# iacopoermacora/Street-sparse-3DGS

Hardware: AMD Instinct MI355X
Metric: fwd+bwd Mpix/s at 1080p (1M Gaussians) (higher is better)
Workload: dtype f32; 1 GPU; rasterizer fwd+bwd, 1000000 Gaussians, SH degree 3, 1920x1080, do_depth; gaussians=1000000, width=1920, height=1080, sh_degree=3, tiles=8160, fwd_segment=2048, parallelism=chunk-per-gpu x1

## Files before the change

street-sparse-3dgs_amd/csrc/dsort.hip:

```cpp
#include "gsr_launch.h"

namespace gsr {

namespace {

constexpr int kDsThreads = 1024;
constexpr int kDsWaves = kDsThreads / kWave;
constexpr int kDsItems = 8;
constexpr int kDsTile = kDsThreads * kDsItems;
constexpr int kDigitBits = 9;
constexpr int kRadix = 1 << kDigitBits;
constexpr int kPasses = 4;
constexpr int kLookWin = 16;
constexpr int kMaxResident = 240;
constexpr uint32_t kKeyBase = 0x3E4CCCCDu;
constexpr uint32_t kTopNarrow = 32u;

constexpr int kCtlTicket = 0;
constexpr int kCtlDone = 4;
constexpr int kCtlK = 5;
constexpr int kCtlErr = 6;
constexpr int kCtlAux = 7;
constexpr int kCtlMaxSB = 8;
constexpr int kCtlFwdReady = 9;
constexpr int kCtlSpare = 10;
constexpr int kCtlCulled = 12;
constexpr int kCtlLive = 13;
constexpr int kCtlWide = 15;
constexpr int kCtlHead = 16;
constexpr int kUpMax = 128;
constexpr int kRowVec = 4;
constexpr int kRowSets = kDsThreads / (kRadix / kRowVec);
constexpr int kRowLoads = kUpMax / kRowSets;
constexpr int kRowGroup = 8;
__host__ __device__ inline int up_tpb(int nb) { return (nb + kUpMax - 1) / kUpMax; }
__host__ __device__ inline int up_blocks(int nb) { return (nb + up_tpb(nb) - 1) / up_tpb(nb); }
__host__ __device__ inline size_t ctl_status(int nb, int p) { return kCtlHead + (size_t)p * nb * kRadix; }
__host__ __device__ inline size_t ctl_zero_words(int nb) { return ctl_status(nb, kPasses); }
__host__ __device__ inline size_t ctl_bex(int nb) { return ctl_zero_words(nb); }
__host__ __device__ inline size_t ctl_btot(int nb) { return ctl_bex(nb) + nb; }
__host__ __device__ inline size_t ctl_blkhist(int nb) { return (ctl_btot(nb) + kUpMax + 63) / 64 * 64; }
__host__ __device__ inline size_t ctl_words(int nb) { return ctl_blkhist(nb) + (size_t)kUpMax * kPasses * kRadix; }
constexpr int kSpinLimit = 1 << 20;

#ifdef GSR_DS_TRACE
__device__ uint64_t *g_ds_trace;
#define DS_STAMP(kern, slot)                                                                          \
    do {                                                                                              \
        if (threadIdx.x == 0) {                                                                       \
            const uint64_t t_ = __builtin_amdgcn_s_memrealtime();                                     \
            __builtin_amdgcn_s_waitcnt(0xC07F);                                                       \
            if (blockIdx.x < 4096) g_ds_trace[((size_t)(kern) * 4096 + blockIdx.x) * 8 + (slot)] = t_; \
        }                                                                                             \
    } while (0)
#else
#define DS_STAMP(kern, slot) \
    do {                     \
    } while (0)
#endif
#ifdef GSR_DS_TRACE
#define DS_STAMP_AFTER(kern, slot, x)            \
    do {                                         \
        asm volatile("s_waitcnt vmcnt(0)" ::"v"(x)); \
        DS_STAMP(kern, slot);                    \
    } while (0)
#else
#define DS_STAMP_AFTER(kern, slot, x) DS_STAMP(kern, slot)
#endif


constexpr uint32_t kFlagAgg = 1u << 30, kFlagInc = 2u << 30, kCountMask = (1u << 30) - 1u;

__device__ __forceinline__ uint32_t ld_agent(const uint32_t *p) {
    return __hip_atomic_load(p, __ATOMIC_RELAXED, __HIP_MEMORY_SCOPE_AGENT);
}
__device__ __forceinline__ void st_agent(uint32_t *p, uint32_t v) {
    __hip_atomic_store(p, v, __ATOMIC_RELAXED, __HIP_MEMORY_SCOPE_AGENT);
}

__device__ __forceinline__ uint32_t below(uint64_t m) {
    return __builtin_amdgcn_mbcnt_hi((uint32_t)(m >> 32), __builtin_amdgcn_mbcnt_lo((uint32_t)m, 0u));
}

template <int p>
__device__ __forceinline__ uint32_t digit_of(uint32_t key) {
    const uint32_t r = key - kKeyBase;
    if (p < kPasses - 1) return (r >> (kDigitBits * p)) & (uint32_t)(kRadix - 1);
    return (r >> (kDigitBits * p)) + (key >= kKeyBase ? kTopNarrow : 0u);
}

__device__ __forceinline__ uint64_t match_digit(uint32_t d, uint64_t valid) {
    uint64_t m = valid;
#pragma unroll
    for (int b = 0; b < kDigitBits; b++) {
        const uint32_t spread = (uint32_t)((int32_t)(d << (31 - b)) >> 31);
        const uint64_t bb = __ballot(spread != 0u);
        m &= ~(bb ^ ((uint64_t)spread << 32 | spread));
    }
    return m;
}

__device__ __forceinline__ uint32_t wave_incl_scan(uint32_t v, int lane) {
#pragma unroll
    for (int o = 1; o < 64; o <<= 1) {
        const uint32_t t = (uint32_t)__shfl_up((int)v, o, 64);
        if (lane >= o) v += t;
    }
    return v;
}

__device__ __forceinline__ uint32_t scan_radix_wave(uint32_t *a, int lane) {
    constexpr int kPer = kRadix / kWave;
    uint32_t x[kPer], s = 0;
#pragma unroll
    for (int k = 0; k < kPer; k++) {
        x[k] = a[kPer * lane + k];
        s += x[k];
    }
    const uint32_t incl = wave_incl_scan(s, lane);
    uint32_t e = incl - s;
#pragma unroll
    for (int k = 0; k < kPer; k++) {
        a[kPer * lane + k] = e;
        e += x[k];
    }
    return (uint32_t)__shfl((int)incl, 63, 64);
}

__global__ __launch_bounds__(kDsThreads) void dsort_upsweep_kernel(int P, int nb, const uint32_t *__restrict__ keys,
                                                                    const uint32_t *__restrict__ tiles,
                                                                    uint32_t *__restrict__ ctl,
                                                                    uint32_t *__restrict__ host_K,
                                                                    uint32_t *__restrict__ host_wide) {
    GSR_KS(kKsUpsweep);
    constexpr int kMidCopies = 16;
    __shared__ uint32_t s_hist[kPasses * kRadix];
    __shared__ uint32_t s_mid[kMidCopies][kRadix];
    __shared__ uint32_t s_wsum[kDsWaves];
    __shared__ uint32_t s_cull, s_far;
    const int t = threadIdx.x, w = t >> 6, lane = t & 63;
    const int u = blockIdx.x, tpb = up_tpb(nb);
    DS_STAMP(0, 0);
#pragma unroll
    for (int k = 0; k < kPasses * kRadix / kDsThreads; k++) s_hist[t + k * kDsThreads] = 0u;
    if (t == 0) s_cull = s_far = 0u;
#pragma unroll
    for (int k = 0; k < kMidCopies * kRadix / kDsThreads; k++) (&s_mid[0][0])[t + k * kDsThreads] = 0u;
    __syncthreads();
    uint32_t run = 0;
    uint32_t culled = 0;
    uint32_t near = 0;
    bool far = false;
    const int v1 = min(nb, (u + 1) * tpb);
    for (int v = u * tpb; v < v1; v++) {
        const size_t base = (size_t)v * kDsTile + (size_t)w * kDsItems * kWave;
        uint32_t key[kDsItems], tl[kDsItems];
#pragma unroll
        for (int k = 0; k < kDsItems; k++) {
            const size_t e = base + (size_t)k * kWave + lane;
            key[k] = e < (size_t)P ? keys[e] : 0u;
            tl[k] = e < (size_t)P ? tiles[e] : 0u;
        }
        uint32_t sum = 0;
#pragma unroll
        for (int k = 0; k < kDsItems; k++) {
            const size_t e = base + (size_t)k * kWave + lane;
            const bool cull = e < (size_t)P && key[k] == 0xFFFFFFFFu;
            const bool vis = e < (size_t)P && !cull;
            const uint32_t top = digit_of<3>(key[k]);
            const uint64_t nearm = __ballot(vis && top == kTopNarrow);
            culled += (uint32_t)__popcll(__ballot(cull));
            near += (uint32_t)__popcll(nearm);
            if (vis) {
                atomicAdd(&s_hist[digit_of<0>(key[k])], 1u);
                atomicAdd(&s_hist[kRadix + digit_of<1>(key[k])], 1u);
                atomicAdd(&s_mid[lane & (kMidCopies - 1)][digit_of<2>(key[k])], 1u);
                if (top != kTopNarrow) atomicAdd(&s_hist[3 * kRadix + top], 1u);
            }
            far = far || __ballot(vis) != nearm;
            sum += tl[k];
        }
#pragma unroll
        for (int o = 32; o > 0; o >>= 1) sum += (uint32_t)__shfl_xor((int)sum, o, 64);
        if (lane == 0) s_wsum[w] = sum;
        __syncthreads();
        if (t == 0) {
            ctl[ctl_bex(nb) + v] = run;
#pragma unroll
            for (int k = 0; k < kDsWaves; k++) run += s_wsum[k];
        }
        __syncthreads();
    }
    if (lane == 0) {
        if (culled) atomicAdd(&s_cull, culled);
        if (near) atomicAdd(&s_hist[3 * kRadix + kTopNarrow], near);
        if (far) s_far = 1u;
    }
    __syncthreads();
    DS_STAMP(0, 1);
#pragma unroll
    for (int k = 0; k < kPasses * kRadix / kDsThreads; k++) {
        const int i = t + k * kDsThreads;
        uint32_t hv = s_hist[i];
        if (i >= 2 * kRadix && i < 3 * kRadix) {
#pragma unroll
            for (int c = 0; c < kMidCopies; c++) hv += s_mid[c][i - 2 * kRadix];
        }
        ctl[ctl_blkhist(nb) + (size_t)u * kPasses * kRadix + i] = hv;
    }
    if (t == 0) {
        ctl[ctl_btot(nb) + u] = run;
        __hip_atomic_fetch_add(&ctl[kCtlK], run, __ATOMIC_RELAXED, __HIP_MEMORY_SCOPE_AGENT);
        if (s_cull) __hip_atomic_fetch_add(&ctl[kCtlCulled], s_cull, __ATOMIC_RELAXED, __HIP_MEMORY_SCOPE_AGENT);
        if (s_far) __hip_atomic_fetch_or(&ctl[kCtlWide], 1u, __ATOMIC_RELAXED, __HIP_MEMORY_SCOPE_AGENT);
        const uint32_t done = __hip_atomic_fetch_add(&ctl[kCtlDone], 1u, __ATOMIC_ACQ_REL, __HIP_MEMORY_SCOPE_AGENT);
        if (done == (uint32_t)gridDim.x - 1u && host_K) {
            const uint32_t K = ld_agent(&ctl[kCtlK]);
            if (host_wide) __hip_atomic_store(host_wide, ld_agent(&ctl[kCtlWide]), __ATOMIC_RELAXED, __HIP_MEMORY_SCOPE_SYSTEM);
            __hip_atomic_store(host_K, K, __ATOMIC_RELEASE, __HIP_MEMORY_SCOPE_SYSTEM);
        }
    }
    DS_STAMP(0, 2);
}

template <int kPass>
__global__ __launch_bounds__(kDsThreads) void dsort_pass_kernel(int P, int nb, const uint32_t *__restrict__ kin,
                                                                 uint32_t *__restrict__ kout,
                                                                 const uint32_t *__restrict__ vin,
                                                                 uint32_t *__restrict__ vout,
                                                                 uint32_t *__restrict__ order, uint32_t *__restrict__ ctl,
                                                                 uint32_t *__restrict__ offsets,
                                                                 const uint32_t *__restrict__ tiles,
                                                                 const uint2 *__restrict__ rect8,
                                                                 const uint32_t *__restrict__ rect4,
                                                                 uint2 *__restrict__ drect,
                                                                 const uint32_t *__restrict__ rin,
                                                                 uint32_t *__restrict__ rout,
                                                                 uint32_t *__restrict__ host_err) {
    GSR_KS(kKsPass0 + kPass);
    constexpr bool kFirst = kPass == 0;
    const bool wide = kPass >= 2 && ctl[kCtlWide] != 0u;
    if (kPass == kPasses - 1 && !wide) return;
    const bool last = kPass == kPasses - 1 || (kPass == kPasses - 2 && !wide);
    const bool carry = rect4 != nullptr;
    __shared__ uint32_t s_key[kDsTile];
    __shared__ uint32_t s_val[kDsTile];
    __shared__ uint32_t s_rc[kDsTile];
    __shared__ uint32_t s_wh[kDsWaves][kRadix];
    __shared__ __attribute__((aligned(16))) uint32_t s_gb[kRowSets][kRadix];
    __shared__ uint32_t s_bex[kRadix];
    __shared__ uint32_t s_dst[kRadix];
    __shared__ uint32_t s_wsum[kDsWaves];
    __shared__ uint32_t s_v, s_pre, s_nsort;
    const int t = threadIdx.x, w = t >> 6, lane = t & 63;
    DS_STAMP(1 + kPass, 0);
#pragma unroll
    for (int k = 0; k < kDsWaves * kRadix / kDsThreads; k++) (&s_wh[0][0])[t + k * kDsThreads] = 0u;
    const int nbu = up_blocks(nb);
    const uint4 *bh = reinterpret_cast<const uint4 *>(ctl + ctl_blkhist(nb) + kPass * kRadix) + (t & (kRadix / kRowVec - 1));
    const auto row = [&](int q) {
        const int j = t / (kRadix / kRowVec) + kRowSets * q;
        return j < nbu ? bh[(size_t)j * (kPasses * kRadix / kRowVec)] : make_uint4(0u, 0u, 0u, 0u);
    };
    constexpr int kRowGroups = kRowLoads / kRowGroup, kRowEvery = kDsItems / kRowGroups;
    static_assert(kRowLoads % kRowGroup == 0 && kDsItems % kRowGroups == 0, "row groups spread over the ranked items");
    uint4 h[kRowGroup], gsum = make_uint4(0u, 0u, 0u, 0u);
    const auto sum_rows = [&]() {
#pragma unroll
        for (int q = 0; q < kRowGroup; q++) {
            gsum.x += h[q].x;
            gsum.y += h[q].y;
            gsum.z += h[q].z;
            gsum.w += h[q].w;
        }
    };
#pragma unroll
    for (int q = 0; q < kRowGroup; q++) h[q] = row(q);
    uint32_t v = blockIdx.x;
    if (nb > kMaxResident) {
        if (t == 0) s_v = atomicAdd(&ctl[kCtlTicket + kPass], 1u);
        __syncthreads();
        v = s_v;
    } else {
        __builtin_amdgcn_s_waitcnt(0xc07f);
        __builtin_amdgcn_s_barrier();
    }
    const size_t Pn = kFirst ? (size_t)P : (size_t)P - min((size_t)ctl[kCtlCulled], (size_t)P);
    const uint32_t nbv = (uint32_t)((Pn + kDsTile - 1) / kDsTile);
    if (v >= nbv) return;
    DS_STAMP(1 + kPass, 5);
    const int wbase = w * kDsItems * kWave;
    const size_t tile0 = (size_t)v * kDsTile;
    const int n = (int)min((size_t)kDsTile, Pn - tile0);
    uint32_t key[kDsItems], val[kDsItems], tl[kDsItems];
#pragma unroll
    for (int k = 0; k < kDsItems; k++) {
        const int i = wbase + k * kWave + lane;
        const bool valid = i < n;
        key[k] = valid ? kin[tile0 + i] : 0xFFFFFFFFu;
        val[k] = (!kFirst && valid) ? vin[tile0 + i] : 0u;
        tl[k] = (kFirst && valid) ? tiles[tile0 + i] : 0u;
    }
    DS_STAMP_AFTER(1 + kPass, 6, key[kDsItems - 1] + val[kDsItems - 1]);
    if (kFirst) {
        if (w == 0) {
            const int u = (int)v / up_tpb(nb);
            uint32_t c = 0;
#pragma unroll
            for (int q = 0; q < kUpMax / kWave; q++) c += lane + q * kWave < u ? ctl[ctl_btot(nb) + lane + q * kWave] : 0u;
#pragma unroll
            for (int o = 32; o > 0; o >>= 1) c += (uint32_t)__shfl_xor((int)c, o, 64);
            if (lane == 0) s_pre = c + ctl[ctl_bex(nb) + v];
        }
        uint32_t run = 0;
#pragma unroll
        for (int k = 0; k < kDsItems; k++) {
            const uint32_t incl = wave_incl_scan(tl[k], lane);
            s_key[wbase + k * kWave + lane] = run + incl - tl[k];
            run += (uint32_t)__shfl((int)incl, 63, 64);
        }
        if (lane == 0) s_wsum[w] = run;
    }
    uint32_t rk[kDsItems];
#pragma unroll
    for (int k = 0; k < kDsItems; k++) {
        const bool valid = wbase + k * kWave + lane < n && key[k] != 0xFFFFFFFFu;
        const uint32_t d = digit_of<kPass>(key[k]) & (uint32_t)(kRadix - 1);
        const uint64_t m = match_digit(d, __ballot(valid));
        const uint32_t b = below(m);
        const uint32_t old = s_wh[w][d];
        if (valid && b == 0u) s_wh[w][d] = old + (uint32_t)__popcll(m);
        rk[k] = old + b;
        if ((k + 1) % kRowEvery == 0 && (k + 1) / kRowEvery < kRowGroups) {
            asm volatile("" ::: "memory");
            sum_rows();
#pragma unroll
            for (int q = 0; q < kRowGroup; q++) h[q] = row((k + 1) / kRowEvery * kRowGroup + q);
        }
    }
    sum_rows();
    *reinterpret_cast<uint4 *>(&s_gb[t / (kRadix / kRowVec)][kRowVec * (t & (kRadix / kRowVec - 1))]) = gsum;
    uint32_t rc[kDsItems];
    if (carry) {
        const uint32_t *rsrc = kFirst ? rect4 : rin;
#pragma unroll
        for (int k = 0; k < kDsItems; k++) {
            const int i = wbase + k * kWave + lane;
            rc[k] = i < n ? rsrc[tile0 + i] : 0u;
        }
    }
    __syncthreads();
    DS_STAMP(1 + kPass, 1);
    if (kFirst) {
        uint32_t pre = s_pre;
        for (int k = 0; k < w; k++) pre += s_wsum[k];
#pragma unroll
        for (int k = 0; k < kDsItems; k++) {
            const int i = wbase + k * kWave + lane;
            if (i < n) offsets[tile0 + i] = pre + s_key[i];
        }
    }
    uint32_t cnt = 0;
    if (t < kRadix) {
#pragma unroll
        for (int ww = 0; ww < kDsWaves; ww++) {
            const uint32_t c = s_wh[ww][t];
            s_wh[ww][t] = cnt;
            cnt += c;
        }
        uint32_t *st = ctl + ctl_status(nb, kPass);
        st_agent(&st[(size_t)v * kRadix + t], (v == 0 ? kFlagInc : kFlagAgg) | cnt);
        s_bex[t] = cnt;
        uint32_t gb = s_gb[0][t];
#pragma unroll
        for (int q = 1; q < kRowSets; q++) gb += s_gb[q][t];
        s_gb[0][t] = gb;
    }
    __syncthreads();
    if (w == 0) {
        const uint32_t nv = scan_radix_wave(s_bex, lane);
        if (lane == 0) s_nsort = nv;
    }
    if (w == 1) (void)scan_radix_wave(s_gb[0], lane);
    __syncthreads();
    const int nsort = (int)s_nsort;
    DS_STAMP(1 + kPass, 2);
    int wb = wbase + lane;
    asm volatile("" : "+v"(wb));
#pragma unroll
    for (int k = 0; k < kDsItems; k++) {
        const int i = wb + k * kWave;
        if (i < n && key[k] != 0xFFFFFFFFu) {
            const uint32_t d = digit_of<kPass>(key[k]) & (uint32_t)(kRadix - 1);
            const uint32_t lp = s_bex[d] + s_wh[w][d] + rk[k];
            s_key[lp] = key[k];
            s_val[lp] = kFirst ? (uint32_t)tile0 + (uint32_t)i : val[k];
            if (carry) s_rc[lp] = rc[k];
        }
    }
    DS_STAMP(1 + kPass, 7);
    if (t < kRadix) {
        const uint32_t *st = ctl + ctl_status(nb, kPass);
        uint32_t excl = 0;
        int spins = 0;
        for (int j = (int)v - 1; j >= 0;) {
            uint32_t s[kLookWin];
#pragma unroll
            for (int q = 0; q < kLookWin; q++)
                s[q] = j - q >= 0 ? ld_agent(&st[(size_t)(j - q) * kRadix + t]) : kFlagInc;
            int q = 0;
            bool inc = false;
#pragma unroll
            for (int qq = 0; qq < kLookWin; qq++) {
                const uint32_t f = s[qq] & ~kCountMask;
                if (q == qq && f != 0u && !inc) {
                    excl += s[qq] & kCountMask;
                    inc = f == kFlagInc;
                    q = qq + 1;
                }
            }
            if (inc) break;
            j -= q;
            if (q < kLookWin) {
                if (++spins > kSpinLimit) {
                    ctl[kCtlErr] = 1u;
                    if (host_err) __hip_atomic_store(host_err, 1u, __ATOMIC_RELAXED, __HIP_MEMORY_SCOPE_SYSTEM);
                    break;
                }
                __builtin_amdgcn_s_sleep(1);
            }
        }
        if (v > 0) st_agent(&ctl[ctl_status(nb, kPass) + (size_t)v * kRadix + t], kFlagInc | (excl + cnt));
        s_dst[t] = s_gb[0][t] + excl - s_bex[t];
    }
    __syncthreads();
    DS_STAMP(1 + kPass, 3);
    for (int i = t; i < nsort; i += kDsThreads) {
        const uint32_t k = s_key[i];
        const uint32_t j = s_dst[digit_of<kPass>(k) & (uint32_t)(kRadix - 1)] + (uint32_t)i;
        const uint32_t g = s_val[i];
        if (last) {
            order[j] = g;
            if (carry) reinterpret_cast<uint32_t *>(drect)[j] = s_rc[i];
            else drect[j] = rect8[g];
        } else {
            kout[j] = k;
            vout[j] = g;
            if (carry) rout[j] = s_rc[i];
        }
    }
    DS_STAMP(1 + kPass, 4);
}

}

int dsort_blocks(int P) { return (P + kDsTile - 1) / kDsTile; }

size_t dsort_ctrl_words(int P) { return ctl_words(dsort_blocks(P) > 0 ? dsort_blocks(P) : 1); }
size_t dsort_ctrl_zero_words(int P) { return ctl_zero_words(dsort_blocks(P) > 0 ? dsort_blocks(P) : 1); }

void launch_depth_sort(int P, const GeomState &gs, uint32_t *host_K, uint32_t *host_wide, uint32_t *host_err,
                       hipStream_t s, hipEvent_t k_ready) {
    if (P == 0) return;
    const int nb = dsort_blocks(P);
    hipLaunchKernelGGL(dsort_upsweep_kernel, dim3(up_blocks(nb)), dim3(kDsThreads), 0, s, P, nb, gs.dkey, gs.tiles,
                       gs.ctrl, host_K, host_wide);
    if (k_ready) (void)hipEventRecord(k_ready, s);
    uint32_t *ra = reinterpret_cast<uint32_t *>(gs.rect8), *rb = ra + P;
    hipLaunchKernelGGL(dsort_pass_kernel<0>, dim3(nb), dim3(kDsThreads), 0, s, P, nb, gs.dkey, gs.dkey_sorted,
                       (const uint32_t *)nullptr, gs.ids, (uint32_t *)nullptr, gs.ctrl, gs.offsets, gs.tiles, gs.rect8,
                       gs.rect4, gs.drect, (const uint32_t *)nullptr, ra, host_err);
    hipLaunchKernelGGL(dsort_pass_kernel<1>, dim3(nb), dim3(kDsThreads), 0, s, P, nb, gs.dkey_sorted, gs.dkey, gs.ids,
                       gs.ids2, (uint32_t *)nullptr, gs.ctrl, gs.offsets, gs.tiles, gs.rect8, gs.rect4, gs.drect, ra,
                       rb, host_err);
    hipLaunchKernelGGL(dsort_pass_kernel<2>, dim3(nb), dim3(kDsThreads), 0, s, P, nb, gs.dkey, gs.dkey_sorted, gs.ids2,
                       gs.ids, gs.order, gs.ctrl, gs.offsets, gs.tiles, gs.rect8, gs.rect4, gs.drect, rb, ra, host_err);
    hipLaunchKernelGGL(dsort_pass_kernel<3>, dim3(nb), dim3(kDsThreads), 0, s, P, nb, gs.dkey_sorted,
                       (uint32_t *)nullptr, gs.ids, (uint32_t *)nullptr, gs.order, gs.ctrl, gs.offsets, gs.tiles,
                       gs.rect8, gs.rect4, gs.drect, ra, (uint32_t *)nullptr, host_err);
}

uint32_t *dsort_K_word(const GeomState &gs) { return gs.ctrl + kCtlK; }
uint32_t *dsort_err_word(const GeomState &gs) { return gs.ctrl + kCtlErr; }
uint32_t *dsort_aux_word(const GeomState &gs) { return gs.ctrl + kCtlAux; }
uint32_t *dsort_maxsb_word(const GeomState &gs) { return gs.ctrl + kCtlMaxSB; }
uint32_t *dsort_fwdready_word(const GeomState &gs) { return gs.ctrl + kCtlFwdReady; }
uint32_t *dsort_culled_word(const GeomState &gs) { return gs.ctrl + kCtlCulled; }
uint32_t *dsort_live_words(const GeomState &gs) { return gs.ctrl + kCtlLive; }
int dsort_head_words() { return kCtlHead; }

GSR_KSTAMP_READER(kstamp_read_dsort)

}
```

Measured before the change: 3397 Mpix/s.

## Fold fourth radix pass into third-pass kernel via device-wide phase barrier

Removes the separate launch of the fourth depth-sort pass. When the wide flag is set, the third-pass kernel processes its tiles by ticket, counts finished tiles in a control word, spins until all are done, then processes the fourth pass in the same launch. In the common non-wide case this only removes a launch that would have returned immediately. The cost is a spin barrier that relies on all blocks being able to make progress, plus extra register pinning in the looped path.

Result: no change. 3406 Mpix/s, median of 6 (+0.2%).

```diff
diff --git a/street-sparse-3dgs_amd/csrc/dsort.hip b/street-sparse-3dgs_amd/csrc/dsort.hip
--- a/street-sparse-3dgs_amd/csrc/dsort.hip
+++ b/street-sparse-3dgs_amd/csrc/dsort.hip
@@ -24,6 +24,8 @@
 constexpr int kCtlMaxSB = 8;
 constexpr int kCtlFwdReady = 9;
 constexpr int kCtlSpare = 10;
+constexpr int kCtlPhase = kCtlSpare;
+constexpr int kCtlTicket3 = kCtlSpare + 1;
 constexpr int kCtlCulled = 12;
 constexpr int kCtlLive = 13;
 constexpr int kCtlWide = 15;
@@ -223,36 +225,46 @@
     DS_STAMP(0, 2);
 }
 
-template <int kPass>
-__global__ __launch_bounds__(kDsThreads) void dsort_pass_kernel(int P, int nb, const uint32_t *__restrict__ kin,
-                                                                 uint32_t *__restrict__ kout,
-                                                                 const uint32_t *__restrict__ vin,
-                                                                 uint32_t *__restrict__ vout,
-                                                                 uint32_t *__restrict__ order, uint32_t *__restrict__ ctl,
-                                                                 uint32_t *__restrict__ offsets,
-                                                                 const uint32_t *__restrict__ tiles,
-                                                                 const uint2 *__restrict__ rect8,
-                                                                 const uint32_t *__restrict__ rect4,
-                                                                 uint2 *__restrict__ drect,
-                                                                 const uint32_t *__restrict__ rin,
-                                                                 uint32_t *__restrict__ rout,
-                                                                 uint32_t *__restrict__ host_err) {
-    GSR_KS(kKsPass0 + kPass);
+struct PassLds {
+    uint32_t key[kDsTile];
+    uint32_t val[kDsTile];
+    uint32_t rc[kDsTile];
+    uint32_t wh[kDsWaves][kRadix];
+    __attribute__((aligned(16))) uint32_t gb[kRowSets][kRadix];
+    uint32_t bex[kRadix];
+    uint32_t dst[kRadix];
+    uint32_t wsum[kDsWaves];
+    uint32_t v, pre, nsort;
+};
+
+template <int kPass, bool kLooped>
+__device__ __forceinline__ bool dsort_pass_tile(PassLds &L, const bool last, const bool by_ticket, uint32_t *ticket,
+                                                int P, int nb, const uint32_t *__restrict__ kin,
+                                                uint32_t *__restrict__ kout, const uint32_t *__restrict__ vin,
+                                                uint32_t *__restrict__ vout, uint32_t *__restrict__ order,
+                                                uint32_t *__restrict__ ctl, uint32_t *__restrict__ offsets,
+                                                const uint32_t *__restrict__ tiles, const uint2 *__restrict__ rect8,
+                                                const uint32_t *__restrict__ rect4, uint2 *__restrict__ drect,
+                                                const uint32_t *__restrict__ rin, uint32_t *__restrict__ rout,
+                                                uint32_t *__restrict__ host_err) {
     constexpr bool kFirst = kPass == 0;
-    const bool wide = kPass >= 2 && ctl[kCtlWide] != 0u;
-    if (kPass == kPasses - 1 && !wide) return;
-    const bool last = kPass == kPasses - 1 || (kPass == kPasses - 2 && !wide);
     const bool carry = rect4 != nullptr;
-    __shared__ uint32_t s_key[kDsTile];
-    __shared__ uint32_t s_val[kDsTile];
-    __shared__ uint32_t s_rc[kDsTile];
-    __shared__ uint32_t s_wh[kDsWaves][kRadix];
-    __shared__ __attribute__((aligned(16))) uint32_t s_gb[kRowSets][kRadix];
-    __shared__ uint32_t s_bex[kRadix];
-    __shared__ uint32_t s_dst[kRadix];
-    __shared__ uint32_t s_wsum[kDsWaves];
-    __shared__ uint32_t s_v, s_pre, s_nsort;
-    const int t = threadIdx.x, w = t >> 6, lane = t & 63;
+    auto &s_key = L.key;
+    auto &s_val = L.val;
+    auto &s_rc = L.rc;
+    auto &s_wh = L.wh;
+    auto &s_gb = L.gb;
+    auto &s_bex = L.bex;
+    auto &s_dst = L.dst;
+    auto &s_wsum = L.wsum;
+    uint32_t &s_v = L.v, &s_pre = L.pre, &s_nsort = L.nsort;
+    int t = threadIdx.x;
+    if (kLooped) {
+        asm volatile("" : "+v"(t));
+        asm volatile("" : "+s"(nb));
+        asm volatile("" : "+s"(P));
+    }
+    const int w = t >> 6, lane = t & 63;
     DS_STAMP(1 + kPass, 0);
 #pragma unroll
     for (int k = 0; k < kDsWaves * kRadix / kDsThreads; k++) (&s_wh[0][0])[t + k * kDsThreads] = 0u;
@@ -277,8 +289,8 @@
 #pragma unroll
     for (int q = 0; q < kRowGroup; q++) h[q] = row(q);
     uint32_t v = blockIdx.x;
-    if (nb > kMaxResident) {
-        if (t == 0) s_v = atomicAdd(&ctl[kCtlTicket + kPass], 1u);
+    if (by_ticket) {
+        if (t == 0) s_v = atomicAdd(ticket, 1u);
         __syncthreads();
         v = s_v;
     } else {
@@ -287,7 +299,7 @@
     }
     const size_t Pn = kFirst ? (size_t)P : (size_t)P - min((size_t)ctl[kCtlCulled], (size_t)P);
     const uint32_t nbv = (uint32_t)((Pn + kDsTile - 1) / kDsTile);
-    if (v >= nbv) return;
+    if (v >= nbv) return false;
     DS_STAMP(1 + kPass, 5);
     const int wbase = w * kDsItems * kWave;
     const size_t tile0 = (size_t)v * kDsTile;
@@ -298,7 +310,7 @@
         const int i = wbase + k * kWave + lane;
         const bool valid = i < n;
         key[k] = valid ? kin[tile0 + i] : 0xFFFFFFFFu;
-        val[k] = (!kFirst && valid) ? vin[tile0 + i] : 0u;
+        val[k] = (!kFirst && !kLooped && valid) ? vin[tile0 + i] : 0u;
         tl[k] = (kFirst && valid) ? tiles[tile0 + i] : 0u;
     }
     DS_STAMP_AFTER(1 + kPass, 6, key[kDsItems - 1] + val[kDsItems - 1]);
@@ -341,6 +353,14 @@
     sum_rows();
     *reinterpret_cast<uint4 *>(&s_gb[t / (kRadix / kRowVec)][kRowVec * (t & (kRadix / kRowVec - 1))]) = gsum;
     uint32_t rc[kDsItems];
+    if (kLooped && !kFirst) {
+        asm volatile("" ::: "memory");
+#pragma unroll
+        for (int k = 0; k < kDsItems; k++) {
+            const int i = wbase + k * kWave + lane;
+            val[k] = i < n ? vin[tile0 + i] : 0u;
+        }
+    }
     if (carry) {
         const uint32_t *rsrc = kFirst ? rect4 : rin;
 #pragma unroll
@@ -439,6 +459,7 @@
         const uint32_t k = s_key[i];
         const uint32_t j = s_dst[digit_of<kPass>(k) & (uint32_t)(kRadix - 1)] + (uint32_t)i;
         const uint32_t g = s_val[i];
+        if (kPass == kPasses - 1 && j >= (uint32_t)Pn) continue;
         if (last) {
             order[j] = g;
             if (carry) reinterpret_cast<uint32_t *>(drect)[j] = s_rc[i];
@@ -450,6 +471,68 @@
         }
     }
     DS_STAMP(1 + kPass, 4);
+    return true;
+}
+
+__device__ __forceinline__ void dsort_wide_phases(PassLds &L, int P, int nb, const uint32_t *kin, uint32_t *kout,
+                                                  const uint32_t *vin, uint32_t *vout, uint32_t *order, uint32_t *ctl,
+                                                  const uint2 *rect8, const uint32_t *rect4, uint2 *drect,
+                                                  const uint32_t *rin, uint32_t *rout, uint32_t *host_err) {
+    constexpr int kPass = kPasses - 2;
+    while (dsort_pass_tile<kPass, true>(L, false, true, &ctl[kCtlTicket + kPass], P, nb, kin, kout, vin, vout, nullptr, ctl,
+                                        nullptr, nullptr, rect8, rect4, nullptr, rin, rout, host_err)) {
+        asm volatile("s_waitcnt vmcnt(0)" ::: "memory");
+        __syncthreads();
+        if (threadIdx.x == 0) {
+            __builtin_amdgcn_fence(__ATOMIC_RELEASE, "agent");
+            asm volatile("s_waitcnt vmcnt(0)" ::: "memory");
+            __hip_atomic_fetch_add(&ctl[kCtlPhase], 1u, __ATOMIC_RELAXED, __HIP_MEMORY_SCOPE_AGENT);
+        }
+    }
+    if (threadIdx.x == 0) {
+        const uint32_t nbv = (uint32_t)(((size_t)P - min((size_t)ctl[kCtlCulled], (size_t)P) + kDsTile - 1) / kDsTile);
+        int spins = 0;
+        while (ld_agent(&ctl[kCtlPhase]) < nbv) {
+            if (++spins > kSpinLimit) {
+                ctl[kCtlErr] = 1u;
+                if (host_err) __hip_atomic_store(host_err, 1u, __ATOMIC_RELAXED, __HIP_MEMORY_SCOPE_SYSTEM);
+                break;
+            }
+            __builtin_amdgcn_s_sleep(1);
+        }
+        __builtin_amdgcn_fence(__ATOMIC_ACQUIRE, "agent");
+        asm volatile("s_waitcnt vmcnt(0)" ::: "memory");
+    }
+    __syncthreads();
+    while (dsort_pass_tile<kPasses - 1, true>(L, true, true, &ctl[kCtlTicket3], P, nb, kout, nullptr, vout, nullptr, order,
+                                              ctl, nullptr, nullptr, rect8, rect4, drect, rout, nullptr, host_err)) {
+    }
+}
+
+template <int kPass>
+__global__ __launch_bounds__(kDsThreads) void dsort_pass_kernel(int P, int nb, const uint32_t *__restrict__ kin,
+                                                                 uint32_t *__restrict__ kout,
+                                                                 const uint32_t *__restrict__ vin,
+                                                                 uint32_t *__restrict__ vout,
+                                                                 uint32_t *__restrict__ order, uint32_t *__restrict__ ctl,
+                                                                 uint32_t *__restrict__ offsets,
+                                                                 const uint32_t *__restrict__ tiles,
+                                                                 const uint2 *__restrict__ rect8,
+                                                                 const uint32_t *__restrict__ rect4,
+                                                                 uint2 *__restrict__ drect,
+                                                                 const uint32_t *__restrict__ rin,
+                                                                 uint32_t *__restrict__ rout,
+                                                                 uint32_t *__restrict__ host_err) {
+    static_assert(kPass < kPasses - 1, "pass 3 has no launch of its own");
+    GSR_KS(kKsPass0 + kPass);
+    __shared__ PassLds L;
+    constexpr bool kThird = kPass == kPasses - 2;
+    if (kThird && ctl[kCtlWide] != 0u) {
+        dsort_wide_phases(L, P, nb, kin, kout, vin, vout, order, ctl, rect8, rect4, drect, rin, rout, host_err);
+        return;
+    }
+    (void)dsort_pass_tile<kPass, false>(L, kThird, nb > kMaxResident, &ctl[kCtlTicket + kPass], P, nb, kin, kout, vin, vout,
+                                 order, ctl, offsets, tiles, rect8, rect4, drect, rin, rout, host_err);
 }
 
 }
@@ -475,9 +558,6 @@
                        rb, host_err);
     hipLaunchKernelGGL(dsort_pass_kernel<2>, dim3(nb), dim3(kDsThreads), 0, s, P, nb, gs.dkey, gs.dkey_sorted, gs.ids2,
                        gs.ids, gs.order, gs.ctrl, gs.offsets, gs.tiles, gs.rect8, gs.rect4, gs.drect, rb, ra, host_err);
-    hipLaunchKernelGGL(dsort_pass_kernel<3>, dim3(nb), dim3(kDsThreads), 0, s, P, nb, gs.dkey_sorted,
-                       (uint32_t *)nullptr, gs.ids, (uint32_t *)nullptr, gs.order, gs.ctrl, gs.offsets, gs.tiles,
-                       gs.rect8, gs.rect4, gs.drect, ra, (uint32_t *)nullptr, host_err);
 }
 
 uint32_t *dsort_K_word(const GeomState &gs) { return gs.ctrl + kCtlK; }
```
